# OHDSI/bayes-bridge

Measured on AMD Instinct MI355X. Metric: Gibbs iters/sec (cg sampler), higher is better.
Workload: dtype f64

## Files before the change

### bayes-bridge_amd/bayesbridge_amd/_lib.py

```python
import ctypes
import os
from ctypes import (POINTER, byref, c_char_p, c_double, c_int, c_int32,
                    c_int64, c_uint64, c_void_p)

_HERE = os.path.dirname(os.path.abspath(__file__))
LIB_PATH = os.path.join(os.path.dirname(_HERE), "libbbx.so")

ABI_VERSION = 113
FORMAT_AUTO, FORMAT_CSR, FORMAT_TILED = 0, 1, 2
F64, F32 = 0, 1
MODEL_LINEAR, MODEL_LOGIT = 0, 1
GSCALE_SAMPLE, GSCALE_OPTIMIZE, GSCALE_FIXED = 0, 1, 2
BATCH_ALLOW_SLOW = 1
ERR_NUMERIC = -4
SAMPLER_CG, SAMPLER_CHOLESKY, SAMPLER_WOODBURY = 0, 1, 2
STREAM_ETA1, STREAM_ETA2 = 1, 2

_lib = None
finalizing = False


def _mark_finalizing():
    global finalizing
    finalizing = True
# ... 42 lines not shown
        "bbx_design_format": ([hp, POINTER(c_int)], c_int),
        "bbx_design_storage_bytes": ([hp, POINTER(c_int64)], c_int),
        "bbx_design_matvec_bytes": (
            [hp, POINTER(c_int64), POINTER(c_int64)], c_int),
        "bbx_design_useful_bytes": (
            [hp, POINTER(c_int64), POINTER(c_int64), POINTER(c_double),
             POINTER(c_double)], c_int),
        "bbx_design_timed_bytes": (
            [hp, POINTER(c_int64), POINTER(c_int64)], c_int),
        "bbx_design_fused_operator_bytes": ([hp, POINTER(c_int64)], c_int),
        "bbx_design_cg_launches": ([hp, POINTER(c_int)], c_int),
        "bbx_design_cg_stats": ([hp, POINTER(c_int64), POINTER(c_int64),
                                 POINTER(c_int64), c_int], c_int),
        "bbx_launch_count": ([], c_uint64),
        "bbx_design_set_cg_fold": ([hp, c_int], c_int),
        "bbx_design_hybrid_info": (
            [hp, POINTER(c_int), POINTER(c_int64), POINTER(c_int64),
             POINTER(c_int64), POINTER(c_int)], c_int),
        "bbx_design_tiled_info": (
            [hp, c_int, POINTER(c_int), POINTER(c_int), POINTER(c_int),
             POINTER(c_int), POINTER(c_int64), POINTER(c_int64),
             POINTER(c_int)], c_int),
        "bbx_design_dot": ([hp, c_void_p, c_void_p], c_int),
        "bbx_design_tdot": ([hp, c_void_p, c_void_p], c_int),
        "bbx_design_dot_dev": ([hp, c_void_p, c_void_p], c_int),
        "bbx_design_tdot_dev": ([hp, c_void_p, c_void_p], c_int),
        "bbx_design_gram_matvec": ([hp, c_void_p, c_void_p, c_void_p], c_int),
        "bbx_design_gram_matvec_dev": (
            [hp, c_void_p, c_void_p, c_void_p], c_int),
        "bbx_design_fisher_info": ([hp, c_void_p, c_int, c_void_p], c_int),
# ... 36 lines not shown
        "bbx_design_reset_timing": ([hp], c_int),
        "bbx_hbm_probe": (
            [c_int, c_int64, c_int, POINTER(c_double), POINTER(c_double)],
            c_int),
        "bbx_chain_create": (
            [hp, c_int, c_void_p, c_void_p, c_int, c_void_p, c_double,
             c_double, c_double, c_double, c_uint64, POINTER(hp)], c_int),
        "bbx_chain_destroy": ([hp], c_int),
        "bbx_chain_set_state": (
            [hp, c_void_p, c_void_p, c_void_p, c_void_p], c_int),
        "bbx_chain_get_state": (
            [hp, c_void_p, c_void_p, c_void_p, c_void_p], c_int),
        "bbx_chain_set_summary": ([hp, c_void_p, c_void_p, c_int64], c_int),
        "bbx_chain_get_summary": (
            [hp, c_void_p, c_void_p, POINTER(c_int64)], c_int),
        "bbx_chain_init_obs_prec": ([hp], c_int),
        "bbx_chain_get_iteration": ([hp, POINTER(c_int64)], c_int),
        "bbx_chain_set_iteration": ([hp, c_int64], c_int),
        "bbx_chain_get_seed": ([hp, POINTER(c_uint64)], c_int),
        "bbx_chain_set_seed": ([hp, c_uint64], c_int),
        "bbx_chain_set_gscale_update": ([hp, c_int], c_int),
        "bbx_chain_set_coef_sampler": ([hp, c_int], c_int),
        "bbx_chol_release": ([hp], c_int),
        "bbx_chain_eta": ([hp, c_int64, c_void_p, c_void_p], c_int),
        "bbx_chain_get_logp": (
            [hp, POINTER(c_double), POINTER(c_double)], c_int),
        "bbx_chain_run": (
            [hp, c_int, c_int, c_int, c_int, c_double, c_void_p, c_void_p,
             c_void_p, c_void_p, c_void_p, c_void_p], c_int),
        "bbx_chain_set_progress": ([hp, c_int, c_void_p, c_void_p], c_int),
# ... 143 lines not shown
```

### bayes-bridge_amd/bayesbridge_amd/design_matrix.py

```python
import ctypes
import warnings
from ctypes import byref, c_double, c_int, c_int64, c_void_p

import numpy as np
import scipy.sparse as sparse

from . import _lib


def _ptr(a):
    return None if a is None else a.ctypes.data_as(c_void_p)


def remove_intercept_indicator(X):
    n_rows = X.shape[0]
    if sparse.issparse(X):
        first = np.asarray(X.mean(axis=0)).ravel()
        second = np.asarray(X.multiply(X).mean(axis=0)).ravel()
        variance = second - first ** 2
    else:
        variance = np.var(X, axis=0)
    constant = variance < n_rows * 2. ** -52
    if constant.any():
        warnings.warn(
# ... 88 lines not shown
        from ctypes import c_int
        v = c_int()
        _lib.check(self._lib.bbx_design_cg_launches(self._h, byref(v)))
        return int(v.value)

    def cg_stats(self, reset=False):
        from ctypes import c_int64
        a, b, c = c_int64(), c_int64(), c_int64()
        _lib.check(self._lib.bbx_design_cg_stats(
            self._h, byref(a), byref(b), byref(c), 1 if reset else 0))
        return int(a.value), int(b.value), int(c.value)

    def set_cg_fold(self, on):
        _lib.check(self._lib.bbx_design_set_cg_fold(
            self._h, -1 if on is None else int(bool(on))))

    @property
    def fused_operator_bytes(self):
        v = c_int64()
        _lib.check(self._lib.bbx_design_fused_operator_bytes(self._h,
                                                              byref(v)))
        return int(v.value)

    def tiled_info(self, chains=1):
        out = {}
        base = {1: 0, 2: 2, 4: 4}[int(chains)]
        n, P = self.shape
        for which, name in ((base, 'X'), (base + 1, 'Xt')):
            W, nb, PR, G = c_int(), c_int(), c_int(), c_int()
            nq, ns = c_int64(), c_int64()
# ... 319 lines not shown
```

### bayes-bridge_amd/bayesbridge_amd/device_chain.py

```python
from ctypes import byref, c_double, c_int64, c_uint64, c_void_p

import numpy as np

from . import _lib

_GSCALE_MODES = {'sample': _lib.GSCALE_SAMPLE, 'optimize': _lib.GSCALE_OPTIMIZE,
                 None: _lib.GSCALE_FIXED}


def _ptr(a):
    return None if a is None else a.ctypes.data_as(c_void_p)


def _f64(a):
    return np.ascontiguousarray(a, dtype=np.float64)


class HipGibbsChain():

    def __init__(self, design, family, outcome, n_trial=None,
                 sd_unshrunk=(float('inf'),), bridge_exponent=.5,
                 slab_size=float('inf'), gscale_shape=0., gscale_rate=0.,
                 seed=0):
        if family not in ('linear', 'logit'):
# ... 54 lines not shown
            raise ValueError("local_scale must have length %d" % self.n_shrunk)
        g = None if global_scale is None else c_double(float(global_scale))
        _lib.check(self._lib.bbx_chain_set_state(
            self._c, _ptr(coef), _ptr(obs), _ptr(ls),
            None if g is None else byref(g)))

    def get_state(self):
        coef = np.empty(self.P)
        ls = np.empty(self.n_shrunk)
        obs = np.empty(self._obs_len)
        g = c_double()
        _lib.check(self._lib.bbx_chain_get_state(
            self._c, _ptr(coef), _ptr(obs), _ptr(ls), byref(g)))
        return (coef, obs if self.family == 'logit' else float(obs[0]), ls,
                float(g.value))

    def init_obs_prec(self):
        _lib.check(self._lib.bbx_chain_init_obs_prec(self._c))

    def set_summary(self, mean, square, n_averaged):
        mean, square = _f64(mean), _f64(square)
        if mean.shape != (self.P,) or square.shape != (self.P,):
            raise ValueError("summaries must have length %d" % self.P)
        _lib.check(self._lib.bbx_chain_set_summary(
            self._c, _ptr(mean), _ptr(square), int(n_averaged)))

    def get_summary(self):
        mean, square, n_avg = np.empty(self.P), np.empty(self.P), c_int64()
        _lib.check(self._lib.bbx_chain_get_summary(
            self._c, _ptr(mean), _ptr(square), byref(n_avg)))
# ... 198 lines not shown
```

### bayes-bridge_amd/csrc/api.hip

```cpp
#include <algorithm>
#include <cmath>
#include <cstring>
#include <new>

#include <fcntl.h>
#include <sys/file.h>
#include <unistd.h>

#include <condition_variable>
#include <mutex>
#include <thread>
#include <unordered_set>

#include "common.hpp"
#include "tiled_layout.hpp"

namespace bbx {

static thread_local std::string g_last_error;

void set_error(const std::string& msg) { g_last_error = msg; }
int fail(int code, const std::string& msg) {
  g_last_error = msg;
  return code;
// ... 1354 lines not shown
    BBX_TRY(matvec_bytes_impl(h, true, &db, &tb));
  }
  if (dot_bytes) *dot_bytes = db;
  if (tdot_bytes) *tdot_bytes = tb;
  if (pad_dot) *pad_dot = pd;
  if (pad_tdot) *pad_tdot = pt;
  return BBX_OK;
}

int bbx_design_set_cg_fold(bbx_design* h, int on) {
  BBX_TRY(check_handle(h));
  h->cg_fold = on < 0 ? -1 : (on ? 1 : 0);
  return BBX_OK;
}

uint64_t bbx_launch_count(void) {
  return bbx::g_launch_count.load(std::memory_order_relaxed);
}

int bbx_design_cg_stats(bbx_design* h, int64_t* solves, int64_t* empty_launches,
                        int64_t* naps, int reset) {
  BBX_TRY(check_handle(h));
  if (solves) *solves = h->cg_solves;
  if (empty_launches) *empty_launches = h->cg_empty_launches;
  if (naps) *naps = h->cg_naps;
  if (reset) h->cg_solves = h->cg_empty_launches = h->cg_naps = 0;
  return BBX_OK;
}

int bbx_design_cg_launches(const bbx_design* h, int* per_iteration) {
// ... 31 lines not shown
```

### bayes-bridge_amd/csrc/cg_sampler.hip

```cpp
#include <sys/prctl.h>
#include <time.h>

#include "common.hpp"
#include "philox.hpp"
#include "tiled_layout.hpp"

namespace bbx {

int launch_cg_setup(bbx_design* h, int n_unshrunk, const double* phi,
                    const double* sd, const double* x0, double* s, double* d,
                    double* xs, CGState* st, double atol);
int launch_cg_direction(bbx_design* h, int k, CGState* st,
                        const double* rr_part, const double* r, double* pvec,
                        const double* s, double* sp, double* c_part,
                        const double* d = nullptr, double* pdp_part = nullptr,
                        unsigned long long* word = nullptr,
                        unsigned long long tag = 0);
int launch_cg_update(bbx_design* h, int k, CGState* st, const double* pq_part,
                     const double* pvec, const double* q, double* x, double* r,
                     double* rr_part);
int launch_cg_finish(bbx_design* h, const double* s, const double* x,
                     double* coef);

__global__ __launch_bounds__(256) void fill_normal_kernel(
// ... 70 lines not shown
    const int st = launch_operator_dense_fused(
        h, sp, d_omega, ep, q, upd ? part_slot(h, PS_TWT) : nullptr);
    if (st < 0) return st;
    if (st == 0) return timer_end(h, 2);
    return fail(BBX_ERR_STATE, "single-pass dense operator refused its design");
  }
  double* t = h->w_n[0].as<double>();
  int twt_done = 0;
  BBX_TRY(launch_dot(h, sp, d_omega, t, part_slot(h, PS_SUMW),
                     upd ? part_slot(h, PS_TWT) : nullptr, &twt_done));
  if (upd && twt_done) merge();
  BBX_TRY(launch_tdot(h, t, part_slot(h, PS_SUMW), ep, q));
  return timer_end(h, 2);
}

int cg_sample_device(bbx_design* h, const double* d_omega, const double* d_phi,
                     const double* d_z, const double* d_x0,
                     const double* d_sd, int n_unshrunk, const double* d_eta1,
                     const double* d_eta2, uint64_t seed, int maxiter,
                     double atol, double* d_coef, int* n_iter_out,
                     int* info_out, int x0_zero) {
  if (maxiter < 0) return fail(BBX_ERR_INVALID, "maxiter must be >= 0");
  if (n_unshrunk < 0 || n_unshrunk > h->P)
    return fail(BBX_ERR_INVALID, "n_unshrunk out of range");
  if ((d_eta1 == nullptr) != (d_eta2 == nullptr))
    return fail(BBX_ERR_INVALID,
                "randn_n and randn_P must both be given or both be NULL");
  double* s = h->w_P[0].as<double>();
  double* d = h->w_P[1].as<double>();
  double* x = h->w_P[2].as<double>();
  double* r = h->w_P[3].as<double>();
  double* pvec = h->w_P[4].as<double>();
  double* q = h->w_P[5].as<double>();
  double* sp = h->w_P[6].as<double>() + (h->intercept ? 1 : 0);
  CGState* st = h->cg_state.as<CGState>();
  const bool fold = tiled_fold_applies(h);
  double* sr = h->w_P[9].as<double>() + (h->intercept ? 1 : 0);
  double* tu = h->w_n[2].as<double>();

  if (d_eta1 == nullptr) {
    double* e1 = h->w_n[2].as<double>();
    double* e2 = h->w_P[8].as<double>();
    BBX_TRY(launch_fill_normal(h, h->n, seed, STREAM_ETA1, e1));
    BBX_TRY(launch_fill_normal(h, h->P, seed, STREAM_ETA2, e2));
    d_eta1 = e1;
    d_eta2 = e2;
  }

  BBX_TRY(launch_cg_setup(h, n_unshrunk, d_phi, d_sd, d_x0, s, d, x, st, atol));

  CGState* host_st = static_cast<CGState*>(h->host_pinned);
  if (x0_zero < 0) {
    int* d_flag = &st->pad;
    int* h_flag = reinterpret_cast<int*>(host_st);
    BBX_HIP(hipMemsetAsync(d_flag, 0, sizeof(int), h->stream));
    BBX_LAUNCH(any_nonzero_kernel, dim3(NPART), dim3(256), 0,
                       h->stream, h->P, d_x0, d_flag);
    BBX_HIP(hipGetLastError());
    BBX_HIP(hipMemcpyAsync(h_flag, d_flag, sizeof(int), hipMemcpyDeviceToHost,
                           h->stream));
    BBX_HIP(hipStreamSynchronize(h->stream));
    x0_zero = (*h_flag == 0) ? 1 : 0;
  }

// ... 1 lines not shown
    double* w = h->w_n[1].as<double>();
    TdotEpilogue ep;
    ep.mode = TD_RESID;
    ep.s = s;
    ep.d = d;
    ep.x = x0_zero ? nullptr : x;
    ep.z = d_z;
    ep.phi = d_phi;
    ep.eta2 = d_eta2;
    ep.dot_part = part_slot(h, PS_RR);
    if (fold) {
      ep.fold_sr = sr;
      ep.fold_cr_part = part_slot(h, PS_C);
    }
    if (!x0_zero && !h->sparse && dense_fused_applies(h)) {
      BBX_TRY(launch_prep_v(h, x, s, sp, part_slot(h, PS_C)));
      BBX_TRY(launch_sqrt_scale(h, d_omega, d_eta1, w, part_slot(h, PS_SUMW),
                                nullptr, true));
      const int st_f =
          launch_operator_dense_fused(h, sp, d_omega, ep, r, nullptr, w);
      if (st_f != 0)
        return st_f < 0 ? st_f
                        : fail(BBX_ERR_STATE,
                               "single-pass dense operator refused its design");
    } else {
      const double* t0 = nullptr;
      if (!x0_zero) {
        double* t = h->w_n[0].as<double>();
        BBX_TRY(launch_prep_v(h, x, s, sp, part_slot(h, PS_C)));
        BBX_TRY(launch_dot(h, sp, d_omega, t, nullptr));
        t0 = t;
      }
      BBX_TRY(launch_sqrt_scale(h, d_omega, d_eta1, w, part_slot(h, PS_SUMW),
                                t0, t0 == nullptr));
      BBX_TRY(launch_tdot(h, w, part_slot(h, PS_SUMW), ep, r));
    }
  }


  struct SkipScope {
    bbx_design* h;
    ~SkipScope() { h->skip_flag = nullptr; }
  } skip_scope{h};
  h->skip_flag = &st->done;
// ... 16 lines not shown
                               part_slot(h, PS_RR)));
    return BBX_OK;
  };
  auto folded_iteration = [&](int kk) -> int {
    h->timer.cur_tag = kk;
    DotFold fa;
    fa.word = word;
    fa.tag = tag;
    fa.st = st;
    fa.k = kk;
    fa.intercept = h->intercept;
    fa.P = h->P;
    fa.rr_part = part_slot(h, PS_RR);
    fa.cr_part = part_slot(h, PS_C);
    fa.sr = sr;
    fa.tu = tu;
    fa.r = r;
    fa.pvec = pvec;
    fa.d = d;
    fa.pdp_part = pdp;
    BBX_TRY(timer_begin(h, 2));
    BBX_TRY(launch_dot_tiled_fold(h, fa, d_omega, h->w_n[0].as<double>(),
                                  part_slot(h, PS_SUMW), part_slot(h, PS_TWT)));
    TdotEpilogue ep;
    ep.mode = TD_OPER_UPD;
    ep.s = s;
    ep.d = d;
    ep.x = pvec;
    ep.dot_part = part_slot(h, PS_RR);
    ep.cg_x = x;
    ep.cg_r = r;
// ... 146 lines not shown
```

### bayes-bridge_amd/csrc/chain.hip

```cpp
#include <cmath>
#include <new>
#include <vector>

#include "chain.hpp"
#include "philox.hpp"
#include "samplers.hpp"
#include "pg_queue.hpp"

namespace bbx {

__device__ inline double wsum(double x) { return wave_allsum(x); }

__device__ inline double block_total_256(double x) {
  __shared__ double s_w[256 / WAVE];
  x = wsum(x);
  if ((threadIdx.x & (WAVE - 1)) == 0) s_w[threadIdx.x / WAVE] = x;
  __syncthreads();
  double r = 0.;
  if (threadIdx.x == 0)
    for (int k = 0; k < 256 / WAVE; ++k) r += s_w[k];
  __syncthreads();
  return r;
}

__device__ inline double shrunk_scale(double gscale, double lscale,
                                      double slab) {
  const double raw = gscale * lscale;
  const double ratio = raw / slab;
  return raw / sqrt(1. + ratio * ratio);
}

__global__ __launch_bounds__(256) void chain_prior_kernel(
    int64_t P, int nu, int model, double slab, long long n_avg,
    const ChainScalars* __restrict__ sc, const double* __restrict__ lscale,
    const double* __restrict__ sd_unshrunk, const double* __restrict__ mean,
    const double* __restrict__ square, const double* __restrict__ zbase,
    double* __restrict__ phi, double* __restrict__ x0, double* __restrict__ sd,
    double* __restrict__ z, int store_idx, double* __restrict__ samp_gs,
    double* __restrict__ samp_lp) {
  const double g = sc->gscale;
  const double zs = (model == BBX_MODEL_LINEAR) ? sc->obs_prec : 1.;
  if (store_idx >= 0 && blockIdx.x == 0 && threadIdx.x == 0) {
    samp_gs[store_idx] = g;
    samp_lp[store_idx] = sc->logp();
  }
  for (int64_t j = (int64_t)blockIdx.x * 256 + threadIdx.x; j < P;
       j += (int64_t)gridDim.x * 256) {
    double prior_sd, guess = mean[j];
    if (j < nu) {
      prior_sd = sd_unshrunk[j];
    } else {
      prior_sd = shrunk_scale(g, lscale[j - nu], slab);
      guess *= prior_sd;
    }
    phi[j] = 1. / prior_sd;
    x0[j] = guess;
    double est = 1.;
    if (n_avg > 1) {
      const double k = (double)n_avg;
      const double m = mean[j];
      const double var = k / (k - 1.) * (square[j] - m * m);
      const double w = (k - 1.) / (k - 1. + 5.);
      est = sqrt(w * var + (1. - w) * 1.);
    }
    sd[j] = est;
    z[j] = zs * zbase[j];
  }
}

#define BBX_BRANCH_PRIO() do { if (prio) __builtin_amdgcn_s_setprio(3); } while (0)
static int lscale_prio() {
  static const int on = getenv("BBX_LSCALE_PRIO") ? atoi(getenv("BBX_LSCALE_PRIO")) : 1;
  return on;
}
static int branch_prio() {
  static const int on = !(getenv("BBX_BRANCH_PRIO") && atoi(getenv("BBX_BRANCH_PRIO")) == 0);
  return on;
}
__global__ __launch_bounds__(256) void chain_summary_kernel(
    int64_t P, int nu, double slab, long long n_avg,
    const ChainScalars* __restrict__ sc, const double* __restrict__ lscale,
    const double* __restrict__ coef, double* __restrict__ mean,
// ... 394 lines not shown
  if (!on || !h->sparse || h->format != BBX_FORMAT_TILED || h->hybrid) return false;
  int G = 0;
  return tiled_describe(h, 0, nullptr, nullptr, nullptr, &G, nullptr, nullptr) ==
             BBX_OK && G == 1;
}

static int chain_check(const bbx_chain* c) {
  if (!c || !c->h) return fail(BBX_ERR_INVALID, "chain handle is NULL");
  return BBX_OK;
}

static double power_exp_ave_magnitude(double exponent) {
  return std::tgamma(2. / exponent) / std::tgamma(1. / exponent);
}

int chain_pre_draw(bbx_chain* c) {
  bbx_design* h = c->h;
  hipStream_t s = h->stream;
  const int64_t P = h->P, n = h->n;
  ChainScalars* sc = c->scalars.as<ChainScalars>();
  BBX_LAUNCH(chain_prior_kernel, dim3(NPART), dim3(256), 0, s, P,
                     c->n_unshrunk, c->model, c->slab,
                     (long long)c->n_averaged, sc, c->lscale.as<double>(),
                     c->sd_unshrunk.as<double>(), c->mean.as<double>(),
                     c->square.as<double>(), c->zbase.as<double>(),
                     c->phi.as<double>(), c->x0.as<double>(),
                     c->sd.as<double>(), c->z.as<double>(), c->pending_store,
                     c->samp_gscale.as<double>(), c->samp_logp.as<double>());
  c->pending_store = -1;
  if (c->model == BBX_MODEL_LINEAR)
    BBX_LAUNCH(chain_fill_obs_prec_kernel, dim3(grid_for(n, ROW_GRID)),
                       dim3(256), 0, s, n, sc, c->obs_prec.as<double>());
  BBX_HIP(hipGetLastError());
  return BBX_OK;
}

int chain_post_draw(bbx_chain* c, bool have_psi, int phases,
                    bbx_chain* branch_of) {
  bbx_design* h = c->h;
  hipStream_t s = h->stream;
  const int64_t P = h->P, n = h->n;
  const int nu = c->n_unshrunk;
  const int64_t n_shrunk = P - nu;
// ... 104 lines not shown

  launch_err = hipGetLastError();
  if (phases & POST_JOIN) {
    if (fork) {
      BBX_HIP(hipEventRecord(c->ev_join, s_b));
      BBX_HIP(hipStreamWaitEvent(s, c->ev_join, 0));
    }
    c->iter += 1;
  }
  BBX_HIP(launch_err);
  return BBX_OK;
}

static int chain_step(bbx_chain* c, int maxiter, double atol, int* n_cg_iter) {
  const uint64_t it = (uint64_t)c->iter;
  BBX_TRY(chain_pre_draw(c));
  int info = 0;
  const bool have_eta = c->eta_iter == (long long)it && c->eta1_next.ptr;
  if (c->coef_sampler == BBX_SAMPLER_CHOLESKY) {
    bbx_design* h = c->h;
    if (!have_eta) {
      if (!c->eta2_next.ptr)
        BBX_TRY(c->eta2_next.alloc(sizeof(double) * (size_t)h->P));
      BBX_TRY(launch_fill_normal(h, h->P, cg_draw_seed(c, it), STREAM_ETA2,
                                 c->eta2_next.as<double>()));
    }
    const bool linear = c->model == BBX_MODEL_LINEAR;
    const int st = chol_sample_device(
        h, linear ? nullptr : c->obs_prec.as<double>(), 1.,
        linear ? &c->scalars.as<ChainScalars>()->obs_prec : nullptr,
        c->phi.as<double>(), c->z.as<double>(), c->eta2_next.as<double>(),
// ... 40 lines not shown
      h->coef_copy = nullptr;
    }
  } tail_scope{c->h};
  c->h->coef_copy = c->coef_sample;
  if (chain_tail_applies(c)) {
    c->h->tail_hook = chain_tail_hook;
    c->h->tail_ctx = c;
  }

  int st = cg_sample_device(
      c->h, c->obs_prec.as<double>(), c->phi.as<double>(), c->z.as<double>(),
      c->x0.as<double>(), c->sd.as<double>(), c->n_unshrunk,
      have_eta ? c->eta1_next.as<double>() : nullptr,
      have_eta ? c->eta2_next.as<double>() : nullptr,
      cg_draw_seed(c, it), maxiter, atol, c->coef.as<double>(), n_cg_iter,
      &info, c->mean_zero ? 1 : 0);
  c->eta_iter = -1;
  if (st < 0) return st;
  c->mean_zero = false;
  BBX_TRY(chain_post_draw(c, c->h->tail_ran, POST_ALL));
  c->h->tail_ran = false;
  return info;
}

int chain_begin_run(bbx_chain* c, int n_sample) {
  c->pending_store = -1;
  c->coef_sample = nullptr;
  BBX_TRY(c->samp_gscale.alloc(sizeof(double) * (size_t)(n_sample + 1)));
  BBX_TRY(c->samp_logp.alloc(sizeof(double) * (size_t)(n_sample + 1)));
  return BBX_OK;
}
// ... 265 lines not shown
}

int bbx_chain_get_summary(bbx_chain* c, double* mean, double* square,
                          int64_t* n_averaged) {
  BBX_TRY(chain_check(c));
  BBX_HIP(hipSetDevice(c->h->device));
  BBX_HIP(hipStreamSynchronize(c->h->stream));
  const size_t Pb = sizeof(double) * (size_t)c->h->P;
  if (mean) BBX_HIP(hipMemcpy(mean, c->mean.ptr, Pb, hipMemcpyDeviceToHost));
  if (square)
    BBX_HIP(hipMemcpy(square, c->square.ptr, Pb, hipMemcpyDeviceToHost));
  if (n_averaged) *n_averaged = c->n_averaged;
  return BBX_OK;
}

int bbx_chain_get_iteration(bbx_chain* c, int64_t* iteration) {
  BBX_TRY(chain_check(c));
  if (iteration) *iteration = c->iter;
  return BBX_OK;
}

int bbx_chain_set_iteration(bbx_chain* c, int64_t iteration) {
  BBX_TRY(chain_check(c));
  if (iteration < 0) return fail(BBX_ERR_INVALID, "iteration < 0");
  c->iter = iteration;
  c->eta_iter = -1;
  return BBX_OK;
}

int bbx_chain_get_seed(bbx_chain* c, uint64_t* seed) {
// ... 350 lines not shown
```

### bayes-bridge_amd/csrc/chain.hpp

```cpp
#pragma once
#include <cmath>

#include "common.hpp"

namespace bbx {

constexpr int ROW_GRID = 2048;

struct alignas(128) ChainScalars {
  double gscale;
  double logprior;
  double abs_pow_sum;
  long long n_gscale_clamped;
  long long n_lscale_fixed;
  alignas(128) double obs_prec;
  double loglik;
  __host__ __device__ double logp() const { return loglik + logprior; }
};

}

struct bbx_chain {
  bbx_design* h = nullptr;
  int model = BBX_MODEL_LOGIT;
// ... 20 lines not shown
  long long eta_iter = -1;
  bbx::DevMem samp_gscale, samp_logp;
  int pending_store = -1;
  double* coef_sample = nullptr;
  void* pinned = nullptr;
  hipStream_t stream2 = nullptr;
  hipEvent_t ev_join = nullptr;
};

namespace bbx {

inline uint64_t cg_draw_seed(const bbx_chain* c, uint64_t it) {
  return c->seed + 0x9E3779B97F4A7C15ull * (it + 1);
}

int chain_pre_draw(bbx_chain* c);
enum { POST_BRANCH = 1, POST_MAIN = 2, POST_JOIN = 4, POST_ALL = 7 };
int chain_post_draw(bbx_chain* c, bool have_psi, int phases,
                    bbx_chain* branch_of = nullptr);
int chain_begin_run(bbx_chain* c, int n_sample);
int chain_save_sample(bbx_chain* c, int idx, double* d_coef, double* d_lscale,
                      double* d_obs_prec);
int chain_end_run(bbx_chain* c, int n_sample, double* gscale, double* logp);

}
```

### bayes-bridge_amd/csrc/common.hpp

```cpp
#pragma once

#include <hip/hip_runtime.h>
#include <stdint.h>

#include <exception>
#include <new>
#include <string>
#include <vector>

#include "../../include/bbx.h"

#include <atomic>
namespace bbx {
extern std::atomic<unsigned long long> g_launch_count;
}
#define BBX_LAUNCH(...)                                                   \
  do {                                                                    \
    bbx::g_launch_count.fetch_add(1, std::memory_order_relaxed);          \
    hipLaunchKernelGGL(__VA_ARGS__);                                      \
  } while (0)
#define BBX_LAUNCH_EXT(...)                                               \
  do {                                                                    \
    bbx::g_launch_count.fetch_add(1, std::memory_order_relaxed);          \
    hipExtLaunchKernelGGL(__VA_ARGS__);                                   \
// ... 17 lines not shown
  m += dpp_move<0x128>(m);
  m += dpp_move<0x124>(m);
  m += dpp_move<0x122>(m);
  m += dpp_move<0x121>(m);
  return m;
}
__device__ __forceinline__ double lane_value(double v, int src_lane) {
  const int lo = __builtin_amdgcn_readlane(__double2loint(v), src_lane);
  const int hi = __builtin_amdgcn_readlane(__double2hiint(v), src_lane);
  return __hiloint2double(hi, lo);
}
__device__ __forceinline__ double wave_allsum(double x) {
  const double m = row16_allsum(x);
  return (lane_value(m, 0) + lane_value(m, 16)) +
         (lane_value(m, 32) + lane_value(m, 48));
}
#endif

void set_error(const std::string& msg);
int fail(int code, const std::string& msg);

template <class F>
int no_throw(F&& f) noexcept {
  try {
    return f();
  } catch (const std::bad_alloc&) {
    try {
      return fail(BBX_ERR_INVALID, "out of host memory");
    } catch (...) {
      return BBX_ERR_INVALID;
// ... 201 lines not shown
__device__ inline void cg_word_store(unsigned long long* word,
                                     unsigned long long v) {
  __hip_atomic_store(word, v, __ATOMIC_RELEASE, __HIP_MEMORY_SCOPE_SYSTEM);
}

struct DotFold {
  unsigned long long* word = nullptr;
  unsigned long long tag = 0;
  CGState* st = nullptr;
  int k = 0;
  int intercept = 0;
  int64_t P = 0;
  const double* rr_part = nullptr;
  const double* cr_part = nullptr;
  const double* sr = nullptr;
  double* tu = nullptr;
  const double* r = nullptr;
  double* pvec = nullptr;
  const double* d = nullptr;
  double* pdp_part = nullptr;
};

constexpr int DENSE_EPI_MAX = 8;
struct DenseEpi {
  const double* D = nullptr;
  const int32_t* cols = nullptr;
  int kd = 0;
  int64_t n = 0;
  double* part = nullptr;
};

// ... 111 lines not shown
                           double obs_scalar, const double* d_obs_scalar,
                           const double* d_pps, const double* d_y, int y_is_wy,
                           const double* d_delta, const double* d_xi,
                           double* d_coef_out);
double* wb_stage(bbx_design* h, int k);
void woodbury_release(bbx_design* h);
int launch_dot_dense(bbx_design* h, const double* d_v, const double* d_rowscale,
                     double* d_t);
int launch_tdot_dense(bbx_design* h, const double* d_w, const double* d_sumw_part,
                      const TdotEpilogue& ep, double* d_out);
int cg_sample_device(bbx_design* h, const double* d_omega, const double* d_phi,
                     const double* d_z, const double* d_x0,
                     const double* d_sd, int n_unshrunk, const double* d_eta1,
                     const double* d_eta2, uint64_t seed, int maxiter,
                     double atol, double* d_coef, int* n_iter_out,
                     int* info_out, int x0_zero = -1);

}
```

### bayes-bridge_amd/csrc/spmv_tiled.hip

```cpp
#include <algorithm>
#include <cstdio>
#include <cstring>
#include <thread>

#include <hip/hip_ext.h>

#include "common.hpp"
#include "tiled_layout.hpp"

#ifndef BBX_TILED_INSTRUMENT
#define BBX_TILED_INSTRUMENT 0
#endif
#if BBX_TILED_INSTRUMENT
#define BBX_INSTR_PARAMS int ablate, unsigned long long* dbg,
#define BBX_INSTR_ARGS ablate, dbg,
#else
#define BBX_INSTR_PARAMS
#define BBX_INSTR_ARGS
#endif
#ifndef BBX_EARLY_ISSUE
#define BBX_EARLY_ISSUE 1
#endif
#ifndef BBX_RING_BIN
#define BBX_RING_BIN 3
// ... 724 lines not shown
            if (twt_off)
              out_sum_part[c * part_stride + twt_off + (int)gridDim.x + tid] = 0.;
          }
        }
      }
    } else {
      v2d* dst = reinterpret_cast<v2d*>(slab) + ((int64_t)group * R + row0) * KP;
      for (int r = tid; r < rows_here; r += TILE_THREADS) {
#pragma unroll
        for (int q = 0; q < KP; ++q) dst[(int64_t)r * KP + q] = acc2[q * n_acc + r];
      }
    }
  } else {
    constexpr int EPI_UNROLL = TILE_PR_MAX / TILE_THREADS;
    double rs_pre[EPI_UNROLL];
    double tu_pre[FOLD ? EPI_UNROLL : 1];
    double cp_pre[NPART / WAVE];
    double x0_pre = 0.;
    if (out) {
  #pragma unroll
      for (int u = 0; u < EPI_UNROLL; ++u) {
        const int r = tid + u * TILE_THREADS;
        rs_pre[u] = (rowscale && r < rows_here) ? rowscale[row0 + r] : 1.;
        if constexpr (FOLD)
          tu_pre[u] = (fa.k > 0 && r < rows_here) ? fa.tu[row0 + r] : 0.;
      }
      if constexpr (!FOLD) {
  #pragma unroll
        for (int k = 0; k < NPART / WAVE; ++k)
          cp_pre[k] = c_part ? c_part[lane + k * WAVE] : 0.;
        if (x0_ptr) x0_pre = *x0_ptr;
      }
    }
    __syncthreads();
    {
      const int f0 = panel_fold[panel], f1 = panel_fold[panel + 1];
      for (int f = f0 + tid; f < f1; f += TILE_THREADS) {
        const FoldDesc fd = folds[f];
        double v = acc[fd.row];
        for (int c = 0; c < fd.count; ++c) v += acc[fd.first + c];
// ... 59 lines not shown
          if (lane == 0) s_dw[j * TILE_WAVES + wave] = a;
        }
        __syncthreads();
        if (tid < de.kd) {
          double tot = 0.;
          for (int wv = 0; wv < TILE_WAVES; ++wv) tot += s_dw[tid * TILE_WAVES + wv];
          de.part[(int64_t)bid * de.kd + tid] = tot;
        }
      } else {
  #pragma unroll
      for (int u = 0; u < EPI_UNROLL; ++u) {
        const int r = tid + u * TILE_THREADS;
        if (r < rows_here) {
          double t = c + acc[r];
          if (addend) t += addend[row0 + r];
          if constexpr (FOLD) {
            if (fa.k > 0) t = fma(f_beta, tu_pre[u], t);
            fa.tu[row0 + r] = t;
          }
          double v = t;
          if (rowscale) v *= rs_pre[u];
          out[row0 + r] = v;
          tsum += v;
          t2sum += v * t;
        }
      }
      }
      if (out_sum_part) {
        tsum = wave_allsum(tsum);
        t2sum = wave_allsum(t2sum);
        if constexpr (FOLD) f_pdp = wave_allsum(f_pdp);
        __syncthreads();
        if (lane == 0) {
          xs[wave] = tsum;
          xs[TILE_WAVES + wave] = t2sum;
          if constexpr (FOLD) xs[2 * TILE_WAVES + wave] = f_pdp;
// ... 1396 lines not shown
    int64_t tb = hp->ones.xt.stream_bytes() + dense + 8 * h->n +
                 8 * (int64_t)hp->n_slab * h->p;
    if (hp->rest_nnz > 0) {
      db += hp->rest.x.stream_bytes() + 16 * (int64_t)hp->rest.x.G * h->n + 8 * h->P;
      tb += hp->rest.xt.stream_bytes() + 8 * h->n;
    }
    if (!timed_only) tb += 8 * (int64_t)hp->n_slab * h->p + 8 * h->P;
    *dot_bytes = db;
    *tdot_bytes = tb;
    return BBX_OK;
  }
  const TiledPair* tp = static_cast<const TiledPair*>(h->tiled);
  if (!tp) return fail(BBX_ERR_STATE, "tiled format not built");
  *dot_bytes = tp->x.stream_bytes() + 8 * (h->P + h->n) +
               (tp->x.G > 1 ? 16 * tp->x.G * h->n : 0);
  if (timed_only && tiled_fold_applies(h)) *dot_bytes += 16 * h->n + 4 * 8 * h->P;
  if (timed_only)
    *tdot_bytes = tp->xt.stream_bytes() + 8 * h->n +
                  8 * (int64_t)tp->xt.G * h->p;
  else
    *tdot_bytes = tp->xt.stream_bytes() + 8 * (h->n + h->P) +
                  16 * (int64_t)tp->xt.G * h->p;
  return BBX_OK;
}

int tiled_useful_bytes(const bbx_design* h, int64_t* dot_bytes,
                       int64_t* tdot_bytes, double* pad_dot, double* pad_tdot) {
  const TiledPair* tp = static_cast<const TiledPair*>(h->tiled);
  if (h->hybrid || !tp) return fail(BBX_ERR_STATE, "plain tiled designs only");
  auto ids = [](const TiledMatrix& m, double* pad) {
    const double per_entry = (m.packed ? 1.6 : 2.0) + (m.has_vals ? 8. : 0.);
// ... 67 lines not shown
```

### bayes-bridge_amd/csrc/vecops.hip

```cpp
#include "common.hpp"

namespace bbx {

std::atomic<unsigned long long> g_launch_count{0};


__device__ inline double wave_sum_v(double x) { return wave_allsum(x); }

__device__ inline void block_store_partial(double x, double* part) {
  __shared__ double s_w[VEC_BLOCK / WAVE];
  x = wave_sum_v(x);
  if ((threadIdx.x & (WAVE - 1)) == 0) s_w[threadIdx.x / WAVE] = x;
  __syncthreads();
  if (threadIdx.x == 0) {
    double r = 0.;
#pragma unroll
    for (int k = 0; k < VEC_BLOCK / WAVE; ++k) r += s_w[k];
    part[blockIdx.x] = r;
  }
  __syncthreads();
}

__device__ inline double sum_partials_v(const double* part) {
  __shared__ double s_tot;
  if (threadIdx.x < WAVE) {
    double a = 0.;
#pragma unroll
    for (int k = 0; k < NPART / WAVE; ++k) a += part[threadIdx.x + k * WAVE];
    a = wave_sum_v(a);
    if (threadIdx.x == 0) s_tot = a;
  }
  __syncthreads();
  const double r = s_tot;
  __syncthreads();
  return r;
}
// ... 277 lines not shown
```

### include/bbx.h

```cpp
#ifndef BBX_H
#define BBX_H

#include <stdint.h>

#ifdef __cplusplus
extern "C" {
#endif

#define BBX_VERSION 113

#define BBX_OK 0
#define BBX_ERR_INVALID (-1)
#define BBX_ERR_HIP (-2)
#define BBX_ERR_NODEVICE (-3)
#define BBX_ERR_NUMERIC (-4)
#define BBX_ERR_STATE (-5)

#define BBX_FORMAT_AUTO 0
#define BBX_FORMAT_CSR 1
#define BBX_FORMAT_TILED 2

#define BBX_F64 0
#define BBX_F32 1

// ... 52 lines not shown
int bbx_design_device(const bbx_design* h, int* device);
int bbx_design_format(const bbx_design* h, int* format);
int bbx_design_storage_bytes(const bbx_design* h, int64_t* bytes);
int bbx_design_matvec_bytes(const bbx_design* h, int64_t* dot_bytes,
                            int64_t* tdot_bytes);
int bbx_design_timed_bytes(const bbx_design* h, int64_t* dot_bytes,
                           int64_t* tdot_bytes);
int bbx_design_useful_bytes(const bbx_design* h, int64_t* dot_bytes,
                            int64_t* tdot_bytes, double* pad_dot,
                            double* pad_tdot);
int bbx_design_cg_launches(const bbx_design* h, int* per_iteration);
int bbx_design_cg_stats(bbx_design* h, int64_t* solves, int64_t* empty_launches,
                        int64_t* naps, int reset);
uint64_t bbx_launch_count(void);
int bbx_design_set_cg_fold(bbx_design* h, int on);
int bbx_design_fused_operator_bytes(const bbx_design* h, int64_t* bytes);

int bbx_design_hybrid_info(const bbx_design* h, int* is_hybrid,
                           int64_t* ones_nnz, int64_t* rest_nnz,
                           int64_t* dense_nnz, int* dense_cols);
int bbx_design_tiled_info(const bbx_design* h, int which, int* W,
                          int* n_block, int* PR, int* G, int64_t* n_quad,
                          int64_t* n_slice, int* packed);

int bbx_design_dot(bbx_design* h, const double* v, double* out);
int bbx_design_tdot(bbx_design* h, const double* w, double* out);
int bbx_design_dot_dev(bbx_design* h, const double* d_v, double* d_out);
int bbx_design_tdot_dev(bbx_design* h, const double* d_w, double* d_out);

int bbx_design_gram_matvec(bbx_design* h, const double* obs_prec,
// ... 71 lines not shown
                     const double* n_trial, int n_unshrunk,
                     const double* sd_unshrunk, double bridge_exp,
                     double slab_size, double gscale_shape0,
                     double gscale_rate0, uint64_t seed, bbx_chain** out);
int bbx_chain_destroy(bbx_chain* c);

int bbx_chain_set_state(bbx_chain* c, const double* coef,
                        const double* obs_prec, const double* lscale,
                        const double* gscale);
int bbx_chain_get_state(bbx_chain* c, double* coef, double* obs_prec,
                        double* lscale, double* gscale);
int bbx_chain_set_summary(bbx_chain* c, const double* mean,
                          const double* square, int64_t n_averaged);
int bbx_chain_get_summary(bbx_chain* c, double* mean, double* square,
                          int64_t* n_averaged);
int bbx_chain_init_obs_prec(bbx_chain* c);
int bbx_chain_get_iteration(bbx_chain* c, int64_t* iteration);
int bbx_chain_set_iteration(bbx_chain* c, int64_t iteration);
int bbx_chain_get_seed(bbx_chain* c, uint64_t* seed);
int bbx_chain_set_seed(bbx_chain* c, uint64_t seed);
int bbx_chain_set_gscale_update(bbx_chain* c, int mode);
#define BBX_SAMPLER_CG 0
#define BBX_SAMPLER_CHOLESKY 1
#define BBX_SAMPLER_WOODBURY 2
int bbx_chain_set_coef_sampler(bbx_chain* c, int sampler);
int bbx_chain_eta(bbx_chain* c, int64_t iteration, double* eta1, double* eta2);
int bbx_chain_get_logp(bbx_chain* c, double* loglik, double* logp);

int bbx_chain_run(bbx_chain* c, int n_iter, int n_burnin, int thin,
                  int maxiter, double atol, double* d_coef, double* d_lscale,
// ... 290 lines not shown
```

Baseline: 332.6.

## Fuse CG setup and prep into chain prior kernel; drop tu scratch in fold epilogue

The per-iteration prior kernel now also computes the CG preconditioner scale, diagonal, scaled initial guess, prepared vector and offset partial sums, and initialises the CG state. The separate cg_setup and prep_v launches are skipped when the chain takes the CG path. Separately, the folded tiled SpMV epilogue no longer writes and reads a tu scratch vector over n. It reconstructs t from the previous output divided by the row scale, which saves one n-length read and write but adds a division and depends on the output buffer still holding the prior value.

```diff
diff --git a/bayes-bridge_amd/bayesbridge_amd/_lib.py b/bayes-bridge_amd/bayesbridge_amd/_lib.py
--- a/bayes-bridge_amd/bayesbridge_amd/_lib.py
+++ b/bayes-bridge_amd/bayesbridge_amd/_lib.py
@@ -80,6 +80,7 @@
                                  POINTER(c_int64), c_int], c_int),
         "bbx_launch_count": ([], c_uint64),
         "bbx_design_set_cg_fold": ([hp, c_int], c_int),
+        "bbx_design_cg_workspace": ([hp, c_int, c_void_p], c_int),
         "bbx_design_hybrid_info": (
             [hp, POINTER(c_int), POINTER(c_int64), POINTER(c_int64),
              POINTER(c_int64), POINTER(c_int)], c_int),
@@ -146,6 +147,9 @@
         "bbx_chain_set_summary": ([hp, c_void_p, c_void_p, c_int64], c_int),
         "bbx_chain_get_summary": (
             [hp, c_void_p, c_void_p, POINTER(c_int64)], c_int),
+        "bbx_chain_cg_setup": (
+            [hp, c_int, c_double, c_void_p, c_void_p, c_void_p, c_void_p],
+            c_int),
         "bbx_chain_init_obs_prec": ([hp], c_int),
         "bbx_chain_get_iteration": ([hp, POINTER(c_int64)], c_int),
         "bbx_chain_set_iteration": ([hp, c_int64], c_int),
diff --git a/bayes-bridge_amd/bayesbridge_amd/design_matrix.py b/bayes-bridge_amd/bayesbridge_amd/design_matrix.py
--- a/bayes-bridge_amd/bayesbridge_amd/design_matrix.py
+++ b/bayes-bridge_amd/bayesbridge_amd/design_matrix.py
@@ -126,6 +126,16 @@
     def set_cg_fold(self, on):
         _lib.check(self._lib.bbx_design_set_cg_fold(
             self._h, -1 if on is None else int(bool(on))))
+
+    _CG_WORKSPACE = {'s': 0, 'd': 1, 'x': 2, 'sx': 3, 'c_part': 4, 'r': 5,
+                     'rr_part': 6}
+
+    def cg_workspace(self, name):
+        which = self._CG_WORKSPACE[name]
+        out = np.empty(256 if name.endswith('_part') else self.shape[1])
+        _lib.check(self._lib.bbx_design_cg_workspace(
+            self._h, which, out.ctypes.data_as(c_void_p)))
+        return out
 
     @property
     def fused_operator_bytes(self):
diff --git a/bayes-bridge_amd/bayesbridge_amd/device_chain.py b/bayes-bridge_amd/bayesbridge_amd/device_chain.py
--- a/bayes-bridge_amd/bayesbridge_amd/device_chain.py
+++ b/bayes-bridge_amd/bayesbridge_amd/device_chain.py
@@ -92,6 +92,13 @@
             self._c, _ptr(coef), _ptr(obs), _ptr(ls), byref(g)))
         return (coef, obs if self.family == 'logit' else float(obs[0]), ls,
                 float(g.value))
+
+    def cg_setup(self, atol=0., fused=True):
+        phi, x0, sd, z = (np.empty(self.P) for _ in range(4))
+        _lib.check(self._lib.bbx_chain_cg_setup(
+            self._c, int(bool(fused)), float(atol), _ptr(phi), _ptr(x0),
+            _ptr(sd), _ptr(z)))
+        return phi, x0, sd, z
 
     def init_obs_prec(self):
         _lib.check(self._lib.bbx_chain_init_obs_prec(self._c))
diff --git a/bayes-bridge_amd/csrc/api.hip b/bayes-bridge_amd/csrc/api.hip
--- a/bayes-bridge_amd/csrc/api.hip
+++ b/bayes-bridge_amd/csrc/api.hip
@@ -1392,6 +1392,28 @@
   return BBX_OK;
 }
 
+int bbx_design_cg_workspace(bbx_design* h, int which, double* out) {
+  BBX_TRY(check_handle(h));
+  if (!out) return fail(BBX_ERR_INVALID, "out is NULL");
+  const CGSetupBufs b = cg_setup_bufs(h);
+  const double* src = nullptr;
+  size_t len = (size_t)h->P;
+  switch (which) {
+    case 0: src = b.s; break;
+    case 1: src = b.d; break;
+    case 2: src = b.xs; break;
+    case 3: src = b.v; break;
+    case 4: src = b.c_part; len = NPART; break;
+    case 5: src = h->w_P[3].as<double>(); break;
+    case 6: src = part_slot(h, PS_RR); len = NPART; break;
+    default: return fail(BBX_ERR_INVALID, "which must be 0 ... 6");
+  }
+  BBX_HIP(hipSetDevice(h->device));
+  BBX_HIP(hipStreamSynchronize(h->stream));
+  BBX_HIP(hipMemcpy(out, src, sizeof(double) * len, hipMemcpyDeviceToHost));
+  return BBX_OK;
+}
+
 uint64_t bbx_launch_count(void) {
   return bbx::g_launch_count.load(std::memory_order_relaxed);
 }
diff --git a/bayes-bridge_amd/csrc/cg_sampler.hip b/bayes-bridge_amd/csrc/cg_sampler.hip
--- a/bayes-bridge_amd/csrc/cg_sampler.hip
+++ b/bayes-bridge_amd/csrc/cg_sampler.hip
@@ -108,12 +108,19 @@
   return timer_end(h, 2);
 }
 
+CGSetupBufs cg_setup_bufs(bbx_design* h) {
+  return CGSetupBufs{h->w_P[0].as<double>(), h->w_P[1].as<double>(),
+                     h->w_P[2].as<double>(),
+                     h->w_P[6].as<double>() + (h->intercept ? 1 : 0),
+                     part_slot(h, PS_C), h->cg_state.as<CGState>()};
+}
+
 int cg_sample_device(bbx_design* h, const double* d_omega, const double* d_phi,
                      const double* d_z, const double* d_x0,
                      const double* d_sd, int n_unshrunk, const double* d_eta1,
                      const double* d_eta2, uint64_t seed, int maxiter,
                      double atol, double* d_coef, int* n_iter_out,
-                     int* info_out, int x0_zero) {
+                     int* info_out, int x0_zero, bool setup_done) {
   if (maxiter < 0) return fail(BBX_ERR_INVALID, "maxiter must be >= 0");
   if (n_unshrunk < 0 || n_unshrunk > h->P)
     return fail(BBX_ERR_INVALID, "n_unshrunk out of range");
@@ -130,7 +137,6 @@
   CGState* st = h->cg_state.as<CGState>();
   const bool fold = tiled_fold_applies(h);
   double* sr = h->w_P[9].as<double>() + (h->intercept ? 1 : 0);
-  double* tu = h->w_n[2].as<double>();
 
   if (d_eta1 == nullptr) {
     double* e1 = h->w_n[2].as<double>();
@@ -141,7 +147,8 @@
     d_eta2 = e2;
   }
 
-  BBX_TRY(launch_cg_setup(h, n_unshrunk, d_phi, d_sd, d_x0, s, d, x, st, atol));
+  if (!setup_done)
+    BBX_TRY(launch_cg_setup(h, n_unshrunk, d_phi, d_sd, d_x0, s, d, x, st, atol));
 
   CGState* host_st = static_cast<CGState*>(h->host_pinned);
   if (x0_zero < 0) {
@@ -173,7 +180,7 @@
       ep.fold_cr_part = part_slot(h, PS_C);
     }
     if (!x0_zero && !h->sparse && dense_fused_applies(h)) {
-      BBX_TRY(launch_prep_v(h, x, s, sp, part_slot(h, PS_C)));
+      if (!setup_done) BBX_TRY(launch_prep_v(h, x, s, sp, part_slot(h, PS_C)));
       BBX_TRY(launch_sqrt_scale(h, d_omega, d_eta1, w, part_slot(h, PS_SUMW),
                                 nullptr, true));
       const int st_f =
@@ -186,7 +193,7 @@
       const double* t0 = nullptr;
       if (!x0_zero) {
         double* t = h->w_n[0].as<double>();
-        BBX_TRY(launch_prep_v(h, x, s, sp, part_slot(h, PS_C)));
+        if (!setup_done) BBX_TRY(launch_prep_v(h, x, s, sp, part_slot(h, PS_C)));
         BBX_TRY(launch_dot(h, sp, d_omega, t, nullptr));
         t0 = t;
       }
@@ -233,7 +240,6 @@
     fa.rr_part = part_slot(h, PS_RR);
     fa.cr_part = part_slot(h, PS_C);
     fa.sr = sr;
-    fa.tu = tu;
     fa.r = r;
     fa.pvec = pvec;
     fa.d = d;
diff --git a/bayes-bridge_amd/csrc/chain.hip b/bayes-bridge_amd/csrc/chain.hip
--- a/bayes-bridge_amd/csrc/chain.hip
+++ b/bayes-bridge_amd/csrc/chain.hip
@@ -28,6 +28,31 @@
   const double raw = gscale * lscale;
   const double ratio = raw / slab;
   return raw / sqrt(1. + ratio * ratio);
+}
+
+struct PriorEntry {
+  double phi, guess, est;
+};
+__device__ __forceinline__ PriorEntry prior_entry(
+    int64_t j, int nu, double g, double slab, long long n_avg,
+    const double* __restrict__ lscale, const double* __restrict__ sd_unshrunk,
+    const double* __restrict__ mean, const double* __restrict__ square) {
+  double prior_sd, guess = mean[j];
+  if (j < nu) {
+    prior_sd = sd_unshrunk[j];
+  } else {
+    prior_sd = shrunk_scale(g, lscale[j - nu], slab);
+    guess *= prior_sd;
+  }
+  double est = 1.;
+  if (n_avg > 1) {
+    const double k = (double)n_avg;
+    const double m = mean[j];
+    const double var = k / (k - 1.) * (square[j] - m * m);
+    const double w = (k - 1.) / (k - 1. + 5.);
+    est = sqrt(w * var + (1. - w) * 1.);
+  }
+  return PriorEntry{1. / prior_sd, guess, est};
 }
 
 __global__ __launch_bounds__(256) void chain_prior_kernel(
@@ -46,26 +71,64 @@
   }
   for (int64_t j = (int64_t)blockIdx.x * 256 + threadIdx.x; j < P;
        j += (int64_t)gridDim.x * 256) {
-    double prior_sd, guess = mean[j];
-    if (j < nu) {
-      prior_sd = sd_unshrunk[j];
-    } else {
-      prior_sd = shrunk_scale(g, lscale[j - nu], slab);
-      guess *= prior_sd;
-    }
-    phi[j] = 1. / prior_sd;
+    const PriorEntry e =
+        prior_entry(j, nu, g, slab, n_avg, lscale, sd_unshrunk, mean, square);
+    phi[j] = e.phi;
+    x0[j] = e.guess;
+    sd[j] = e.est;
+    z[j] = zs * zbase[j];
+  }
+}
+
+__global__ __launch_bounds__(VEC_BLOCK) void chain_cg_setup_kernel(
+    int64_t P, int nu, int model, double slab, long long n_avg,
+    const ChainScalars* __restrict__ sc, const double* __restrict__ lscale,
+    const double* __restrict__ sd_unshrunk, const double* __restrict__ mean,
+    const double* __restrict__ square, const double* __restrict__ zbase,
+    double* __restrict__ phi, double* __restrict__ x0, double* __restrict__ sd,
+    double* __restrict__ z, int store_idx, double* __restrict__ samp_gs,
+    double* __restrict__ samp_lp, int intercept,
+    const double* __restrict__ offset, double* __restrict__ s,
+    double* __restrict__ d, double* __restrict__ xs, double* __restrict__ v,
+    double* __restrict__ c_part, CGState* __restrict__ st, double atol) {
+  const double g = sc->gscale;
+  const double zs = (model == BBX_MODEL_LINEAR) ? sc->obs_prec : 1.;
+  if (blockIdx.x == 0 && threadIdx.x == 0) {
+    if (store_idx >= 0) {
+      samp_gs[store_idx] = g;
+      samp_lp[store_idx] = sc->logp();
+    }
+    st->rho[0] = st->rho[1] = 0.;
+    st->atol = atol;
+    st->bnorm2 = 0.;
+    st->n_iter = 0;
+    st->done = 0;
+    st->bad = 0;
+    st->pad = 0;
+    st->running = 1;
+    st->pad2 = 0;
+  }
+  double acc = 0.;
+  for (int64_t j = (int64_t)blockIdx.x * VEC_BLOCK + threadIdx.x; j < P;
+       j += (int64_t)gridDim.x * VEC_BLOCK) {
+    const PriorEntry e =
+        prior_entry(j, nu, g, slab, n_avg, lscale, sd_unshrunk, mean, square);
+    const double ph = e.phi, guess = e.guess, est = e.est;
+    phi[j] = ph;
     x0[j] = guess;
-    double est = 1.;
-    if (n_avg > 1) {
-      const double k = (double)n_avg;
-      const double m = mean[j];
-      const double var = k / (k - 1.) * (square[j] - m * m);
-      const double w = (k - 1.) / (k - 1. + 5.);
-      est = sqrt(w * var + (1. - w) * 1.);
-    }
     sd[j] = est;
     z[j] = zs * zbase[j];
-  }
+    const double sj = (j < nu) ? 2. * est : 1. / ph;
+    const double sp = sj * ph;
+    s[j] = sj;
+    d[j] = sp * sp;
+    const double xj = guess / sj;
+    xs[j] = xj;
+    const double val = xj * sj;
+    v[j] = val;
+    if (j >= intercept) acc += offset[j - intercept] * val;
+  }
+  block_store_partial(acc, c_part);
 }
 
 #define BBX_BRANCH_PRIO() do { if (prio) __builtin_amdgcn_s_setprio(3); } while (0)
@@ -490,19 +553,33 @@
   return std::tgamma(2. / exponent) / std::tgamma(1. / exponent);
 }
 
-int chain_pre_draw(bbx_chain* c) {
+int chain_pre_draw(bbx_chain* c, const double* cg_atol) {
   bbx_design* h = c->h;
   hipStream_t s = h->stream;
   const int64_t P = h->P, n = h->n;
   ChainScalars* sc = c->scalars.as<ChainScalars>();
-  BBX_LAUNCH(chain_prior_kernel, dim3(NPART), dim3(256), 0, s, P,
-                     c->n_unshrunk, c->model, c->slab,
-                     (long long)c->n_averaged, sc, c->lscale.as<double>(),
-                     c->sd_unshrunk.as<double>(), c->mean.as<double>(),
-                     c->square.as<double>(), c->zbase.as<double>(),
-                     c->phi.as<double>(), c->x0.as<double>(),
-                     c->sd.as<double>(), c->z.as<double>(), c->pending_store,
-                     c->samp_gscale.as<double>(), c->samp_logp.as<double>());
+  if (cg_atol) {
+    const CGSetupBufs b = cg_setup_bufs(h);
+    BBX_LAUNCH(chain_cg_setup_kernel, dim3(NPART), dim3(VEC_BLOCK), 0, s, P,
+                       c->n_unshrunk, c->model, c->slab,
+                       (long long)c->n_averaged, sc, c->lscale.as<double>(),
+                       c->sd_unshrunk.as<double>(), c->mean.as<double>(),
+                       c->square.as<double>(), c->zbase.as<double>(),
+                       c->phi.as<double>(), c->x0.as<double>(),
+                       c->sd.as<double>(), c->z.as<double>(), c->pending_store,
+                       c->samp_gscale.as<double>(), c->samp_logp.as<double>(),
+                       h->intercept, h->offset.as<double>(), b.s, b.d, b.xs,
+                       b.v, b.c_part, b.st, *cg_atol);
+  } else {
+    BBX_LAUNCH(chain_prior_kernel, dim3(NPART), dim3(256), 0, s, P,
+                       c->n_unshrunk, c->model, c->slab,
+                       (long long)c->n_averaged, sc, c->lscale.as<double>(),
+                       c->sd_unshrunk.as<double>(), c->mean.as<double>(),
+                       c->square.as<double>(), c->zbase.as<double>(),
+                       c->phi.as<double>(), c->x0.as<double>(),
+                       c->sd.as<double>(), c->z.as<double>(), c->pending_store,
+                       c->samp_gscale.as<double>(), c->samp_logp.as<double>());
+  }
   c->pending_store = -1;
   if (c->model == BBX_MODEL_LINEAR)
     BBX_LAUNCH(chain_fill_obs_prec_kernel, dim3(grid_for(n, ROW_GRID)),
@@ -637,7 +714,9 @@
 
 static int chain_step(bbx_chain* c, int maxiter, double atol, int* n_cg_iter) {
   const uint64_t it = (uint64_t)c->iter;
-  BBX_TRY(chain_pre_draw(c));
+  const bool cg_draw = c->coef_sampler != BBX_SAMPLER_CHOLESKY &&
+                       c->coef_sampler != BBX_SAMPLER_WOODBURY;
+  BBX_TRY(chain_pre_draw(c, cg_draw ? &atol : nullptr));
   int info = 0;
   const bool have_eta = c->eta_iter == (long long)it && c->eta1_next.ptr;
   if (c->coef_sampler == BBX_SAMPLER_CHOLESKY) {
@@ -708,7 +787,7 @@
       have_eta ? c->eta1_next.as<double>() : nullptr,
       have_eta ? c->eta2_next.as<double>() : nullptr,
       cg_draw_seed(c, it), maxiter, atol, c->coef.as<double>(), n_cg_iter,
-      &info, c->mean_zero ? 1 : 0);
+      &info, c->mean_zero ? 1 : 0, true);
   c->eta_iter = -1;
   if (st < 0) return st;
   c->mean_zero = false;
@@ -1004,6 +1083,22 @@
   return BBX_OK;
 }
 
+int bbx_chain_cg_setup(bbx_chain* c, int fused, double atol, double* phi,
+                       double* x0, double* sd, double* z) {
+  BBX_TRY(chain_check(c));
+  if (c->pending_store >= 0)
+    return fail(BBX_ERR_STATE, "bbx_chain_cg_setup inside a run");
+  BBX_HIP(hipSetDevice(c->h->device));
+  BBX_TRY(chain_pre_draw(c, fused ? &atol : nullptr));
+  BBX_HIP(hipStreamSynchronize(c->h->stream));
+  const size_t Pb = sizeof(double) * (size_t)c->h->P;
+  if (phi) BBX_HIP(hipMemcpy(phi, c->phi.ptr, Pb, hipMemcpyDeviceToHost));
+  if (x0) BBX_HIP(hipMemcpy(x0, c->x0.ptr, Pb, hipMemcpyDeviceToHost));
+  if (sd) BBX_HIP(hipMemcpy(sd, c->sd.ptr, Pb, hipMemcpyDeviceToHost));
+  if (z) BBX_HIP(hipMemcpy(z, c->z.ptr, Pb, hipMemcpyDeviceToHost));
+  return BBX_OK;
+}
+
 int bbx_chain_get_iteration(bbx_chain* c, int64_t* iteration) {
   BBX_TRY(chain_check(c));
   if (iteration) *iteration = c->iter;
diff --git a/bayes-bridge_amd/csrc/chain.hpp b/bayes-bridge_amd/csrc/chain.hpp
--- a/bayes-bridge_amd/csrc/chain.hpp
+++ b/bayes-bridge_amd/csrc/chain.hpp
@@ -58,7 +58,7 @@
   return c->seed + 0x9E3779B97F4A7C15ull * (it + 1);
 }
 
-int chain_pre_draw(bbx_chain* c);
+int chain_pre_draw(bbx_chain* c, const double* cg_atol = nullptr);
 enum { POST_BRANCH = 1, POST_MAIN = 2, POST_JOIN = 4, POST_ALL = 7 };
 int chain_post_draw(bbx_chain* c, bool have_psi, int phases,
                     bbx_chain* branch_of = nullptr);
diff --git a/bayes-bridge_amd/csrc/common.hpp b/bayes-bridge_amd/csrc/common.hpp
--- a/bayes-bridge_amd/csrc/common.hpp
+++ b/bayes-bridge_amd/csrc/common.hpp
@@ -55,6 +55,19 @@
   const double m = row16_allsum(x);
   return (lane_value(m, 0) + lane_value(m, 16)) +
          (lane_value(m, 32) + lane_value(m, 48));
+}
+__device__ inline void block_store_partial(double x, double* part) {
+  __shared__ double s_w[VEC_BLOCK / WAVE];
+  x = wave_allsum(x);
+  if ((threadIdx.x & (WAVE - 1)) == 0) s_w[threadIdx.x / WAVE] = x;
+  __syncthreads();
+  if (threadIdx.x == 0) {
+    double r = 0.;
+#pragma unroll
+    for (int k = 0; k < VEC_BLOCK / WAVE; ++k) r += s_w[k];
+    part[blockIdx.x] = r;
+  }
+  __syncthreads();
 }
 #endif
 
@@ -286,7 +299,6 @@
   const double* rr_part = nullptr;
   const double* cr_part = nullptr;
   const double* sr = nullptr;
-  double* tu = nullptr;
   const double* r = nullptr;
   double* pvec = nullptr;
   const double* d = nullptr;
@@ -428,6 +440,15 @@
                      const double* d_sd, int n_unshrunk, const double* d_eta1,
                      const double* d_eta2, uint64_t seed, int maxiter,
                      double atol, double* d_coef, int* n_iter_out,
-                     int* info_out, int x0_zero = -1);
-
-}
+                     int* info_out, int x0_zero = -1, bool setup_done = false);
+struct CGSetupBufs {
+  double* s;
+  double* d;
+  double* xs;
+  double* v;
+  double* c_part;
+  CGState* st;
+};
+CGSetupBufs cg_setup_bufs(bbx_design* h);
+
+}
diff --git a/bayes-bridge_amd/csrc/spmv_tiled.hip b/bayes-bridge_amd/csrc/spmv_tiled.hip
--- a/bayes-bridge_amd/csrc/spmv_tiled.hip
+++ b/bayes-bridge_amd/csrc/spmv_tiled.hip
@@ -762,7 +762,7 @@
   } else {
     constexpr int EPI_UNROLL = TILE_PR_MAX / TILE_THREADS;
     double rs_pre[EPI_UNROLL];
-    double tu_pre[FOLD ? EPI_UNROLL : 1];
+    double wp_pre[FOLD ? EPI_UNROLL : 1];
     double cp_pre[NPART / WAVE];
     double x0_pre = 0.;
     if (out) {
@@ -771,7 +771,7 @@
         const int r = tid + u * TILE_THREADS;
         rs_pre[u] = (rowscale && r < rows_here) ? rowscale[row0 + r] : 1.;
         if constexpr (FOLD)
-          tu_pre[u] = (fa.k > 0 && r < rows_here) ? fa.tu[row0 + r] : 0.;
+          wp_pre[u] = (fa.k > 0 && r < rows_here) ? out[row0 + r] : 0.;
       }
       if constexpr (!FOLD) {
   #pragma unroll
@@ -861,12 +861,14 @@
         if (r < rows_here) {
           double t = c + acc[r];
           if (addend) t += addend[row0 + r];
-          if constexpr (FOLD) {
-            if (fa.k > 0) t = fma(f_beta, tu_pre[u], t);
-            fa.tu[row0 + r] = t;
-          }
           double v = t;
           if (rowscale) v *= rs_pre[u];
+          if constexpr (FOLD) {
+            if (fa.k > 0) {
+              v = fma(f_beta, wp_pre[u], v);
+              t = v / rs_pre[u];
+            }
+          }
           out[row0 + r] = v;
           tsum += v;
           t2sum += v * t;
@@ -2293,7 +2295,7 @@
   if (!tp) return fail(BBX_ERR_STATE, "tiled format not built");
   *dot_bytes = tp->x.stream_bytes() + 8 * (h->P + h->n) +
                (tp->x.G > 1 ? 16 * tp->x.G * h->n : 0);
-  if (timed_only && tiled_fold_applies(h)) *dot_bytes += 16 * h->n + 4 * 8 * h->P;
+  if (timed_only && tiled_fold_applies(h)) *dot_bytes += 8 * h->n + 4 * 8 * h->P;
   if (timed_only)
     *tdot_bytes = tp->xt.stream_bytes() + 8 * h->n +
                   8 * (int64_t)tp->xt.G * h->p;
diff --git a/bayes-bridge_amd/csrc/vecops.hip b/bayes-bridge_amd/csrc/vecops.hip
--- a/bayes-bridge_amd/csrc/vecops.hip
+++ b/bayes-bridge_amd/csrc/vecops.hip
@@ -7,19 +7,6 @@
 
 __device__ inline double wave_sum_v(double x) { return wave_allsum(x); }
 
-__device__ inline void block_store_partial(double x, double* part) {
-  __shared__ double s_w[VEC_BLOCK / WAVE];
-  x = wave_sum_v(x);
-  if ((threadIdx.x & (WAVE - 1)) == 0) s_w[threadIdx.x / WAVE] = x;
-  __syncthreads();
-  if (threadIdx.x == 0) {
-    double r = 0.;
-#pragma unroll
-    for (int k = 0; k < VEC_BLOCK / WAVE; ++k) r += s_w[k];
-    part[blockIdx.x] = r;
-  }
-  __syncthreads();
-}
 
 __device__ inline double sum_partials_v(const double* part) {
   __shared__ double s_tot;
diff --git a/include/bbx.h b/include/bbx.h
--- a/include/bbx.h
+++ b/include/bbx.h
@@ -90,6 +90,7 @@
                         int64_t* naps, int reset);
 uint64_t bbx_launch_count(void);
 int bbx_design_set_cg_fold(bbx_design* h, int on);
+int bbx_design_cg_workspace(bbx_design* h, int which, double* out);
 int bbx_design_fused_operator_bytes(const bbx_design* h, int64_t* bytes);
 
 int bbx_design_hybrid_info(const bbx_design* h, int* is_hybrid,
@@ -191,6 +192,8 @@
                           const double* square, int64_t n_averaged);
 int bbx_chain_get_summary(bbx_chain* c, double* mean, double* square,
                           int64_t* n_averaged);
+int bbx_chain_cg_setup(bbx_chain* c, int fused, double atol, double* phi,
+                       double* x0, double* sd, double* z);
 int bbx_chain_init_obs_prec(bbx_chain* c);
 int bbx_chain_get_iteration(bbx_chain* c, int64_t* iteration);
 int bbx_chain_set_iteration(bbx_chain* c, int64_t iteration);
```

Result: no change. 331.8 (median of 2 runs) (-0.2%).
